# liuxinren456852/HiDeGS

Measured on AMD Instinct MI355X. Metric: binning-stage iters/sec at 2M Gaussians, 1920x1080 (scan + tile sort + ranges, the built part of the fwd+bwd iteration; the rasterizer fwd/bwd is not built: headline_metric, status), higher is better.
Workload: dtype u64/u32 (binning), f32 (distCUDA2, exchange, masked Adam)

## Files before the change

hidegs_amd/build.py:

```python
from __future__ import annotations

import concurrent.futures as cf
import glob
import hashlib
import os
import shutil
import subprocess
import sys

HERE = os.path.dirname(os.path.abspath(__file__))
CSRC = os.path.join(HERE, "csrc")
INCLUDE = os.path.join(HERE, "..", "include")
OBJDIR = os.path.join(HERE, "build")
LIB = os.path.join(HERE, "libhidegs.so")
VARIANT_DIR = os.path.join(HERE, "variants")
SOURCES = ["abi.cpp", "timing.cpp", "primitives.hip", "knn.hip", "adam.hip", "wire.hip", "rows.hip"]
HEADERS = sorted(glob.glob(os.path.join(CSRC, "*.h"))) + [os.path.join(INCLUDE, "hidegs.h"),
                                                         os.path.join(INCLUDE, "hidegs_rows.h"),
                                                         os.path.join(INCLUDE, "hidegs_resize.h"),
                                                         os.path.join(INCLUDE, "hidegs_clone.h")]

FLAGS = ["--offload-arch=gfx950", "-O3", "-std=c++17", "-fPIC", "-ffp-contract=off", "-Wall",
         "-Wno-unused-function", "-I", INCLUDE]

VARIANTS = {
    "qcap": (["-DHIDEGS_JOB_CAP=64", "-DHIDEGS_MAX_POLLS=65536u"], ["primitives.hip"]),
    "gform": (["-DHIDEGS_QUEUE_MIN=8192"], ["primitives.hip"]),
    "wscout": (["-DHIDEGS_WIDE_SCOUTS=1"], ["primitives.hip"]),
    "pcap": (["-DHIDEGS_PIECE_CAP=16"], ["primitives.hip"]),
}


def hipcc() -> str:
    for cand in (shutil.which("hipcc"), "/opt/rocm/bin/hipcc"):
        if cand and os.path.exists(cand):
            return cand
    raise RuntimeError("hipcc not found: the HIP toolchain is required to build libhidegs.so")


def _command(src: str, obj: str, defines) -> list:
    lang = ["-x", "hip"] if src.endswith(".hip") else []
    return [hipcc(), *FLAGS, *defines, *lang, "-c", src, "-o", obj + ".tmp"]


def _stamp(cmd: list) -> str:
    return hashlib.sha256(" ".join(cmd[1:-2]).encode()).hexdigest()


def _stale(obj: str, src: str, stamp: str) -> bool:
    if not os.path.exists(obj) or not os.path.exists(obj + ".cmd"):
        return True
    with open(obj + ".cmd") as f:
        if f.read().strip() != stamp:
            return True
    t = os.path.getmtime(obj)
    return any(os.path.getmtime(p) > t for p in [src, *HEADERS])


def _compile(src: str, objdir: str, defines, verbose: bool) -> str:
    obj = os.path.join(objdir, os.path.basename(src) + ".o")
    cmd = _command(src, obj, defines)
    stamp = _stamp(cmd)
    if _stale(obj, src, stamp):
        if verbose:
            print(" ".join(cmd), flush=True)
        subprocess.run(cmd, check=True)
        os.replace(obj + ".tmp", obj)
        with open(obj + ".cmd", "w") as f:
            f.write(stamp + "\n")
    return obj


def _link(objs, lib: str, verbose: bool) -> str:
    if not os.path.exists(lib) or any(os.path.getmtime(o) > os.path.getmtime(lib) for o in objs):
        tmp = lib + ".tmp"
        cmd = [hipcc(), "--offload-arch=gfx950", "-shared", "-fPIC", *objs, "-o", tmp]
        if verbose:
            print(" ".join(cmd), flush=True)
        subprocess.run(cmd, check=True)
        os.replace(tmp, lib)
    return lib


ABI_CLIENT_SRC = os.path.join(HERE, "..", "tests", "c_abi", "abi_client.cpp")
ABI_CLIENT = os.path.join(HERE, "..", "tests", "c_abi", "abi_client")


def build_abi_client(verbose: bool = False) -> str:
    deps = [ABI_CLIENT_SRC, LIB, os.path.join(INCLUDE, "hidegs.h")]
    if not os.path.exists(ABI_CLIENT) or any(os.path.getmtime(d) > os.path.getmtime(ABI_CLIENT) for d in deps):
        tmp = ABI_CLIENT + ".tmp"
        cmd = [hipcc(), "--offload-arch=gfx950", "-O2", "-std=c++17", "-ffp-contract=off", "-Wall", ABI_CLIENT_SRC,
               "-L" + HERE, "-lhidegs", "-Wl,-rpath,$ORIGIN/../../hidegs_amd", "-o", tmp]
        if verbose:
            print(" ".join(cmd), flush=True)
        subprocess.run(cmd, check=True)
        os.replace(tmp, ABI_CLIENT)
    return ABI_CLIENT


def variant_path(tag: str) -> str:
    return os.path.join(VARIANT_DIR, f"libhidegs_{tag}.so")


def _compile_all(sources, objdir: str, defines, verbose: bool) -> list:
    os.makedirs(objdir, exist_ok=True)
    with cf.ThreadPoolExecutor(max_workers=8) as ex:
        return list(ex.map(lambda s: _compile(os.path.join(CSRC, s), objdir, defines, verbose), sources))


def build_variant(tag: str, defines, changed=SOURCES, verbose: bool = False) -> str:
    objs = dict(zip(changed, _compile_all(changed, os.path.join(VARIANT_DIR, "obj_" + tag), defines, verbose)))
    rest = [s for s in SOURCES if s not in objs]
    objs.update(zip(rest, _compile_all(rest, OBJDIR, [], verbose)))
    return _link([objs[s] for s in SOURCES], variant_path(tag), verbose)


def build(verbose: bool = False, variants: bool = True) -> str:
    _link(_compile_all(SOURCES, OBJDIR, [], verbose), LIB, verbose)
    if variants:
        with cf.ThreadPoolExecutor(max_workers=len(VARIANTS)) as ex:
            list(ex.map(lambda tv: build_variant(tv[0], *tv[1], verbose=verbose), VARIANTS.items()))
        build_abi_client(verbose)
    return LIB


if __name__ == "__main__":
    print(build(verbose="-v" in sys.argv))
```

hidegs_amd/csrc/primitives.hip:

```cpp
#include "block_scan.h"
#include "common.h"

#include <mutex>

namespace hidegs {
int identify_tile_ranges(const uint64_t* keys, long long n, uint32_t* ranges, int num_tiles, hipStream_t stream);

namespace {

constexpr int kBlock = 256;
constexpr int kItems = 16;
constexpr int kTile = kBlock * kItems;
constexpr int kWavesPerBlock = kBlock / kWave;
constexpr int kRadixBits = 8;
constexpr int kRadix = 1 << kRadixBits;

#ifndef HIDEGS_SCOUTS
#define HIDEGS_SCOUTS 128
#endif

inline int ceil_div(long long a, long long b) { return (int)((a + b - 1) / b); }

#include "scan.h"
#include "radix.h"
#include "segment_forms.h"
#include "queue_trace.h"
#include "hot_queue.h"
#include "segment_sort.h"


constexpr int kRangeKeys = 4;
__global__ __launch_bounds__(kBlock) void identify_ranges_kernel(const uint64_t* __restrict__ keys, long long n,
                                                                 uint2* __restrict__ ranges, uint32_t num_tiles,
                                                                 uint32_t tile_mask)
{
    const long long i0 = ((long long)blockIdx.x * kBlock + threadIdx.x) * kRangeKeys;
    if (i0 >= n) return;
    uint32_t tile[kRangeKeys];
    if (i0 + kRangeKeys <= n && (reinterpret_cast<uintptr_t>(keys) & 15) == 0) {
        const ulonglong2* k2 = reinterpret_cast<const ulonglong2*>(keys + i0);
        const ulonglong2 a = k2[0], b = k2[1];
        tile[0] = (uint32_t)(a.x >> 32) & tile_mask;
        tile[1] = (uint32_t)(a.y >> 32) & tile_mask;
        tile[2] = (uint32_t)(b.x >> 32) & tile_mask;
        tile[3] = (uint32_t)(b.y >> 32) & tile_mask;
    } else {
#pragma unroll
        for (int j = 0; j < kRangeKeys; j++) tile[j] = i0 + j < n ? (uint32_t)(keys[i0 + j] >> 32) & tile_mask : 0u;
    }
    uint32_t prev = i0 == 0 ? 0u : (uint32_t)(keys[i0 - 1] >> 32) & tile_mask;
#pragma unroll
    for (int j = 0; j < kRangeKeys; j++) {
        const long long i = i0 + j;
        if (i >= n) break;
        const uint32_t cur = tile[j];
        if (i == 0) {
            if (cur < num_tiles) ranges[cur].x = 0;
        } else {
            if (cur != prev) {
                if (prev < num_tiles) ranges[prev].y = (uint32_t)i;
                if (cur < num_tiles) ranges[cur].x = (uint32_t)i;
            }
            if (i == n - 1 && cur < num_tiles) ranges[cur].y = (uint32_t)n;
        }
        prev = cur;
    }
}



size_t scan_scratch(long long n)
{
    const int nt = ceil_div(n, kDevScanTile);
    return align_up((size_t)nt * sizeof(uint32_t)) + align_up(sizeof(uint32_t));
}

constexpr int kMaxSegmentBits = 16;
constexpr long long kSegmentedMinN = 65536;
constexpr long long kSegmentedMinAvg = 64;
constexpr long long kTileSegmentedMinAvg = 8;

BigQueue queue_caps(long long n)
{
    BigQueue q{};
    q.rec_cap = (uint32_t)(5 * (n / (kSegCap + 1)) + 8);
#ifdef HIDEGS_JOB_CAP
    q.job_cap = (uint32_t)HIDEGS_JOB_CAP;
#else
    q.job_cap = (uint32_t)(n / 24 + 1024);
#endif
    q.pool_cap = (uint32_t)(n / 2 + 16 * kRadix);
#ifdef HIDEGS_PIECE_CAP
    q.piece_cap = (uint32_t)HIDEGS_PIECE_CAP;
#else
    q.piece_cap = (uint32_t)(n / 512 + 1024);
#endif
    return q;
}

template <typename K>
size_t sort_scratch(long long n)
{
    const int nt = ceil_div(n, kTile);
    size_t b = align_up((size_t)n * sizeof(K)) + align_up((size_t)n * sizeof(uint32_t)) +
               align_up((size_t)kRadix * nt * sizeof(uint32_t)) + 2 * align_up(kRadix * sizeof(uint32_t));
    if (sizeof(K) == 8) {
        const BigQueue q = queue_caps(n);
        b += align_up(sizeof(uint32_t) * (((size_t)1 << kMaxSegmentBits) + 1)) + align_up(kRadix * sizeof(uint32_t)) +
             align_up(Q_WORDS * sizeof(uint32_t)) +
             align_up((size_t)q.rec_cap * sizeof(BigSeg)) + align_up((size_t)q.job_cap * sizeof(uint4)) +
             align_up((size_t)q.pool_cap * sizeof(uint32_t)) + align_up((size_t)q.piece_cap * sizeof(uint2));
    }
    return b;
}

__global__ void identify_ranges_kernel(const uint64_t* __restrict__ keys, long long n, uint2* __restrict__ ranges,
                                       uint32_t num_tiles, uint32_t tile_mask);

template <typename K>
int sort_pairs(void* scratch, size_t scratch_bytes, const K* keys_in, K* keys_out, const uint32_t* vals_in,
               uint32_t* vals_out, long long n, int begin_bit, int end_bit, hipStream_t stream, const char* what,
               uint2* ranges_out = nullptr, int num_tiles = 0)
{
    const int kbits = (int)(8 * sizeof(K));
    if (n < 0 || begin_bit < 0 || end_bit > kbits || begin_bit > end_bit)
        return fail(HIDEGS_E_ARG, std::string(what) + ": bad size or bit range");
    if (n > 0x7fffffffLL) return fail(HIDEGS_E_ARG, std::string(what) + ": more than 2^31-1 items");
    if (n == 0)
        return ranges_out ? identify_tile_ranges(nullptr, 0, reinterpret_cast<uint32_t*>(ranges_out), num_tiles, stream)
                          : 0;
    if (!keys_in || !keys_out || !vals_in || !vals_out)
        return fail(HIDEGS_E_ARG, std::string(what) + ": NULL key/value pointer");
    if (keys_out == keys_in || vals_out == vals_in)
        return fail(HIDEGS_E_ARG, std::string(what) + ": in-place sorting is not supported");
    if (!scratch || scratch_bytes < sort_scratch<K>(n))
        return fail(HIDEGS_E_ARG, std::string(what) + ": scratch buffer too small");

    const int passes = (end_bit - begin_bit + kRadixBits - 1) / kRadixBits;
    if (passes == 0) {
        if (hipMemcpyAsync(keys_out, keys_in, n * sizeof(K), hipMemcpyDeviceToDevice, stream) != hipSuccess ||
            hipMemcpyAsync(vals_out, vals_in, n * sizeof(uint32_t), hipMemcpyDeviceToDevice, stream) != hipSuccess)
            return fail(HIDEGS_E_HIP, std::string(what) + ": copy failed");
        return ranges_out ? identify_tile_ranges(reinterpret_cast<const uint64_t*>(keys_out), n,
                                                 reinterpret_cast<uint32_t*>(ranges_out), num_tiles, stream)
                          : 0;
    }
    const int nt = ceil_div(n, kTile);
    Carver c(scratch);
    K* alt_k = c.take<K>(n);
    uint32_t* alt_v = c.take<uint32_t>(n);
    uint32_t* counts = c.take<uint32_t>((size_t)kRadix * nt);
    uint32_t* totals_pass[2] = {c.take<uint32_t>(kRadix), c.take<uint32_t>(kRadix)};

    const bool avg_ok = ranges_out ? n >= kTileSegmentedMinAvg * (long long)num_tiles
                                   : n >= (kSegmentedMinAvg << (end_bit - 32));
    const bool segmented = sizeof(K) == 8 && begin_bit == 0 && end_bit > 32 && end_bit - 32 <= kMaxSegmentBits &&
                           n >= kSegmentedMinN && avg_ok;
    const int lo_bit = segmented ? 32 : begin_bit;
    const int lsd_passes = segmented ? (end_bit - 32 + kRadixBits - 1) / kRadixBits : passes;

    const bool packed = segmented && ranges_out != nullptr;
    int nseg = 0;
    uint32_t* seg_starts = nullptr;
    uint32_t* low_base = nullptr;
    BigQueue q{};
    if (segmented) {
        nseg = ranges_out ? num_tiles : 1 << (end_bit - 32);
        seg_starts = c.take<uint32_t>(((size_t)1 << kMaxSegmentBits) + 1);
        low_base = c.take<uint32_t>(kRadix);
        q = queue_caps(n);
        q.ctl = c.take<uint32_t>(Q_WORDS);
        q.job = c.take<uint4>(q.job_cap);
        q.rec = c.take<BigSeg>(q.rec_cap);
        q.pool = c.take<uint32_t>(q.pool_cap);
        q.alt_k = reinterpret_cast<uint64_t*>(alt_k);
        q.alt_v = alt_v;
        q.piece = c.take<uint2>(q.piece_cap);
    }

    const K* src_k = keys_in;
    const uint32_t* src_v = vals_in;
    const int span = end_bit - lo_bit;
    int shift = lo_bit;
    int pass_bits[2] = {0, 0};
    for (int p = 0; p < lsd_passes; p++) {
        const int bits = (span * (p + 1)) / lsd_passes - (span * p) / lsd_passes;
        const uint32_t mask = (1u << bits) - 1u;
        const bool to_out = ((lsd_passes - 1 - p) % 2) == 0;
        K* dk = to_out ? keys_out : alt_k;
        uint32_t* dv = to_out ? vals_out : alt_v;
        uint32_t* totals = totals_pass[p & 1];
        const bool last = p == lsd_passes - 1;
        uint4* zero_jobs = segmented && last ? reinterpret_cast<uint4*>(q.ctl) : nullptr;
        static_assert(Q_WORDS * sizeof(uint32_t) % kAlign == 0, "ctl and job slots contiguous");
        const bool rec_in = packed && lsd_passes == 2 && last, rec_digit_out = packed && lsd_passes == 2 && !last;
        const int next_shift = shift + bits;
        const uint32_t next_mask = rec_digit_out ? (1u << (span - bits)) - 1u : 0u;
        const char* hist_name = sizeof(K) == 8 ? "radix_hist_u64" : "radix_hist_u32";
        if (rec_in)
            HIDEGS_LAUNCH(hist_name, (radix_hist_kernel<K, true>), dim3(nt), dim3(kBlock), 0, stream,
                          reinterpret_cast<const K*>(src_v), n, shift, mask, nt, counts, zero_jobs,
                          zero_jobs ? q.job_cap + Q_WORDS / 4 : 0u);
        else
            HIDEGS_LAUNCH(hist_name, radix_hist_kernel<K>, dim3(nt), dim3(kBlock), 0, stream, src_k, n, shift, mask, nt,
                          counts, zero_jobs, zero_jobs ? q.job_cap + Q_WORDS / 4 : 0u);
        const bool low = segmented && last && lsd_passes == 2;
        HIDEGS_LAUNCH("radix_digit_scan", radix_digit_scan_kernel, dim3(mask + 1), dim3(kBlock), 0, stream, counts,
                      nt, totals, low ? totals_pass[0] : nullptr, low ? 1 << pass_bits[0] : 0, low_base);
        if (p < 2) pass_bits[p] = bits;
        const bool with_starts = segmented && last;
        const int b0 = with_starts && lsd_passes == 2 ? pass_bits[0] : 0;
        const bool narrow = (int)mask < kNarrowRadix && n <= kNarrowMaxN && (1 << b0) <= kNarrowRadix;
        const char* scatter_name = sizeof(K) == 8 ? "radix_scatter_u64" : "radix_scatter_u32";
#define HIDEGS_SCATTER(...)                                                                                            \
    HIDEGS_LAUNCH(scatter_name, (radix_scatter_kernel<K, __VA_ARGS__>), dim3(nt), dim3(kSBlock), 0, stream, src_k, src_v, \
                  dk, dv, n, shift, mask, nt, counts, totals, with_starts ? low_base : nullptr, b0,                       \
                  with_starts ? seg_starts : nullptr, next_shift, next_mask)
        if (rec_in) {
            if (narrow) HIDEGS_SCATTER(true, kNarrowRadix, kOutRecords, true);
            else HIDEGS_SCATTER(true, kRadix, kOutRecords, true);
        } else if (rec_digit_out) {
            if (narrow) HIDEGS_SCATTER(false, kNarrowRadix, kOutRecordsDigit);
            else HIDEGS_SCATTER(false, kRadix, kOutRecordsDigit);
        } else if (with_starts && packed) {
            if (narrow) HIDEGS_SCATTER(true, kNarrowRadix, kOutRecords);
            else HIDEGS_SCATTER(true, kRadix, kOutRecords);
        } else if (with_starts) {
            if (narrow) HIDEGS_SCATTER(true, kNarrowRadix);
            else HIDEGS_SCATTER(true, kRadix);
        } else {
            if (narrow) HIDEGS_SCATTER(false, kNarrowRadix);
            else HIDEGS_SCATTER(false, kRadix);
        }
#undef HIDEGS_SCATTER
        src_k = dk;
        src_v = dv;
        shift += bits;
    }
    if (segmented) {
        uint64_t* ko = reinterpret_cast<uint64_t*>(keys_out);
        if (packed)
            HIDEGS_LAUNCH("segment_sort", segment_sort_kernel<true>, dim3(nseg + kScouts), dim3(kBlock), 0, stream, ko,
                          vals_out, seg_starts, ranges_out, nseg, q);
        else
            HIDEGS_LAUNCH("segment_sort", segment_sort_kernel<false>, dim3(nseg + kScouts), dim3(kBlock), 0, stream, ko,
                          vals_out, seg_starts, ranges_out, nseg, q);
        HIDEGS_LAUNCH("big_segments", big_segment_kernel, dim3(kQueueBlocks), dim3(kBlock), 0, stream, ko, vals_out,
                      reinterpret_cast<uint64_t*>(alt_k), alt_v, q);
        const bool debug = debug_enabled();
        uint32_t* async_err = debug ? nullptr : async_error_slot(stream);
        HIDEGS_LAUNCH("piece_sort", piece_sort_kernel, dim3(kPieceBlocks), dim3(kBlock), 0, stream, ko, vals_out,
                      reinterpret_cast<const uint64_t*>(alt_k), alt_v, q, async_err);
        if (debug) {
            if (int rc = check_launch(what, stream, 1)) return rc;
            uint32_t err = 0;
            if (hipMemcpyAsync(&err, q.ctl + kCtlStride * Q_ERROR, sizeof(err), hipMemcpyDeviceToHost, stream) !=
                    hipSuccess ||
                hipStreamSynchronize(stream) != hipSuccess)
                return fail(HIDEGS_E_HIP, std::string(what) + ": queue error readback failed");
            if (err)
                return fail(HIDEGS_E_HIP, std::string(what) + ": hot-tile partition queue error " + std::to_string(err) +
                                              ((err & 1u) ? " (job slots exhausted)" : "") +
                                              ((err & 4u) ? " (a worker gave up waiting)" : "") +
                                              ": the output is not sorted");
        }
    } else if (ranges_out) {
        if (int rc = check_launch(what, stream, 0)) return rc;
        return identify_tile_ranges(reinterpret_cast<const uint64_t*>(keys_out), n,
                                    reinterpret_cast<uint32_t*>(ranges_out), num_tiles, stream);
    }
    return check_launch(what, stream, 0);
}

}

__device__ uint32_t g_queue_error_read;
__global__ void queue_error_take_kernel(int clear)
{
    g_queue_error_read = clear ? __hip_atomic_exchange(&g_queue_error, 0u, __ATOMIC_RELAXED, __HIP_MEMORY_SCOPE_AGENT)
                               : __hip_atomic_load(&g_queue_error, __ATOMIC_RELAXED, __HIP_MEMORY_SCOPE_AGENT);
}

int queue_error(hipStream_t stream, int clear, uint32_t* flags)
{
    static std::mutex m;
    std::lock_guard<std::mutex> lock(m);
    uint32_t v = 0;
    hipLaunchKernelGGL(queue_error_take_kernel, dim3(1), dim3(1), 0, stream, clear);
    if (hipGetLastError() != hipSuccess ||
        hipMemcpyFromSymbolAsync(&v, HIP_SYMBOL(g_queue_error_read), sizeof(v), 0, hipMemcpyDeviceToHost, stream) !=
            hipSuccess ||
        hipStreamSynchronize(stream) != hipSuccess)
        return fail(HIDEGS_E_HIP, "queue_error: readback failed");
    if (clear) v |= take_async_bits(stream);
    *flags = v;
    return 0;
}

int inclusive_scan_u32(void* scratch, size_t scratch_bytes, const uint32_t* in, uint32_t* out, long long n,
                       hipStream_t stream)
{
    if (n < 0) return fail(HIDEGS_E_ARG, "inclusive_scan_u32: negative size");
    if (n == 0) return 0;
    if (!in || !out) return fail(HIDEGS_E_ARG, "inclusive_scan_u32: NULL pointer");
    if (!scratch || scratch_bytes < scan_scratch(n)) return fail(HIDEGS_E_ARG, "inclusive_scan_u32: scratch too small");
    const int nt = ceil_div(n, kDevScanTile);
    Carver c(scratch);
    uint32_t* sums = c.take<uint32_t>(nt);
    HIDEGS_LAUNCH("scan_reduce", scan_reduce_kernel, dim3(nt), dim3(kBlock), 0, stream, in, n, sums);
    const int own = nt <= kOwnOffsetTiles;
    if (!own)
        HIDEGS_LAUNCH("scan_small", scan_small_kernel, dim3(1), dim3(kBlock), 0, stream, sums, nt, (uint32_t*)nullptr);
    HIDEGS_LAUNCH("scan_downsweep", scan_downsweep_kernel, dim3(nt), dim3(kBlock), 0, stream, in, n, sums, own, out);
    return check_launch("inclusive_scan_u32", stream, 0);
}

size_t inclusive_scan_scratch(long long n) { return scan_scratch(n); }
size_t sort_u64_scratch(long long n) { return sort_scratch<uint64_t>(n); }
size_t sort_u32_scratch(long long n) { return sort_scratch<uint32_t>(n); }

int sort_pairs_u64(void* scratch, size_t bytes, const uint64_t* ki, uint64_t* ko, const uint32_t* vi, uint32_t* vo,
                   long long n, int b, int e, hipStream_t s)
{
    return sort_pairs<uint64_t>(scratch, bytes, ki, ko, vi, vo, n, b, e, s, "sort_pairs_u64");
}
int sort_pairs_u32(void* scratch, size_t bytes, const uint32_t* ki, uint32_t* ko, const uint32_t* vi, uint32_t* vo,
                   long long n, int b, int e, hipStream_t s)
{
    return sort_pairs<uint32_t>(scratch, bytes, ki, ko, vi, vo, n, b, e, s, "sort_pairs_u32");
}

int sort_tile_pairs(void* scratch, size_t bytes, const uint64_t* ki, uint64_t* ko, const uint32_t* vi, uint32_t* vo,
                    long long n, int num_tiles, uint32_t* ranges, hipStream_t s)
{
    if (num_tiles < 1) return fail(HIDEGS_E_ARG, "sort_tile_pairs: num_tiles must be >= 1");
    if (!ranges) return fail(HIDEGS_E_ARG, "sort_tile_pairs: NULL ranges");
    const int end = 32 + (int)(32u - (uint32_t)__builtin_clz((uint32_t)num_tiles | 1u));
    if (end > 64) return fail(HIDEGS_E_ARG, "sort_tile_pairs: too many tiles");
    return sort_pairs<uint64_t>(scratch, bytes, ki, ko, vi, vo, n, 0, end, s, "sort_tile_pairs",
                                reinterpret_cast<uint2*>(ranges), num_tiles);
}

int identify_tile_ranges(const uint64_t* keys, long long n, uint32_t* ranges, int num_tiles, hipStream_t stream)
{
    if (n < 0 || num_tiles < 0) return fail(HIDEGS_E_ARG, "identify_tile_ranges: negative size");
    if (num_tiles > 0 && !ranges) return fail(HIDEGS_E_ARG, "identify_tile_ranges: NULL ranges");
    if (num_tiles > 0 && hipMemsetAsync(ranges, 0, (size_t)num_tiles * 2 * sizeof(uint32_t), stream) != hipSuccess)
        return fail(HIDEGS_E_HIP, "identify_tile_ranges: memset failed");
    if (n == 0) return check_launch("identify_tile_ranges", stream, 0);
    if (!keys) return fail(HIDEGS_E_ARG, "identify_tile_ranges: NULL keys");
    HIDEGS_LAUNCH("identify_ranges", identify_ranges_kernel, dim3(ceil_div(n, kBlock * kRangeKeys)), dim3(kBlock), 0, stream, keys, n,
                       reinterpret_cast<uint2*>(ranges), (uint32_t)num_tiles, 0xffffffffu);
    return check_launch("identify_tile_ranges", stream, 0);
}

}

extern "C" {

size_t hidegs_scan_scratch_bytes(long long n) { return n > 0 ? hidegs::inclusive_scan_scratch(n) : 0; }
int hidegs_inclusive_scan_u32(void* scratch, size_t scratch_bytes, const uint32_t* in, uint32_t* out, long long n,
                              void* stream)
{
    if (int rc = hidegs::take_async_error("hidegs_inclusive_scan_u32", hidegs::as_stream(stream))) return rc;
    return hidegs::inclusive_scan_u32(scratch, scratch_bytes, in, out, n, hidegs::as_stream(stream));
}

size_t hidegs_sort_pairs_u64_scratch_bytes(long long n) { return n > 0 ? hidegs::sort_u64_scratch(n) : 0; }
int hidegs_sort_pairs_u64(void* scratch, size_t scratch_bytes, const uint64_t* keys_in, uint64_t* keys_out,
                          const uint32_t* vals_in, uint32_t* vals_out, long long n, int begin_bit, int end_bit,
                          void* stream)
{
    if (int rc = hidegs::take_async_error("hidegs_sort_pairs_u64", hidegs::as_stream(stream))) return rc;
    return hidegs::sort_pairs_u64(scratch, scratch_bytes, keys_in, keys_out, vals_in, vals_out, n, begin_bit, end_bit,
                                  hidegs::as_stream(stream));
}

size_t hidegs_sort_pairs_u32_scratch_bytes(long long n) { return n > 0 ? hidegs::sort_u32_scratch(n) : 0; }
int hidegs_sort_pairs_u32(void* scratch, size_t scratch_bytes, const uint32_t* keys_in, uint32_t* keys_out,
                          const uint32_t* vals_in, uint32_t* vals_out, long long n, int begin_bit, int end_bit,
                          void* stream)
{
    if (int rc = hidegs::take_async_error("hidegs_sort_pairs_u32", hidegs::as_stream(stream))) return rc;
    return hidegs::sort_pairs_u32(scratch, scratch_bytes, keys_in, keys_out, vals_in, vals_out, n, begin_bit, end_bit,
                                  hidegs::as_stream(stream));
}

int hidegs_sort_tile_pairs(void* scratch, size_t scratch_bytes, const uint64_t* keys_in, uint64_t* keys_out,
                           const uint32_t* vals_in, uint32_t* vals_out, long long n, int num_tiles, uint32_t* ranges,
                           void* stream)
{
    if (int rc = hidegs::take_async_error("hidegs_sort_tile_pairs", hidegs::as_stream(stream))) return rc;
    return hidegs::sort_tile_pairs(scratch, scratch_bytes, keys_in, keys_out, vals_in, vals_out, n, num_tiles, ranges,
                                   hidegs::as_stream(stream));
}

int hidegs_identify_tile_ranges(const uint64_t* sorted_keys, long long n, uint32_t* ranges, int num_tiles,
                                void* stream)
{
    if (int rc = hidegs::take_async_error("hidegs_identify_tile_ranges", hidegs::as_stream(stream))) return rc;
    return hidegs::identify_tile_ranges(sorted_keys, n, ranges, num_tiles, hidegs::as_stream(stream));
}

int hidegs_queue_error(void* stream, int clear, uint32_t* flags)
{
    if (!flags) return hidegs::fail(HIDEGS_E_ARG, "hidegs_queue_error: NULL flags");
    return hidegs::queue_error(hidegs::as_stream(stream), clear, flags);
}

uint32_t hidegs_higher_msb(uint32_t n)
{
    uint32_t bits = 32u - (uint32_t)__builtin_clz(n | 1u);
    return bits;
}

#ifdef HIDEGS_QUEUE_TRACE
int hidegs_debug_wide_trace(unsigned long long* host, int max_jobs)
{
    return hidegs::trace_take(hidegs::g_wtrace, hidegs::g_wtrace_n, host, max_jobs);
}

int hidegs_debug_queue_trace(unsigned long long* host, int max_jobs)
{
    return hidegs::trace_take(hidegs::g_qtrace, hidegs::g_qtrace_n, host, max_jobs);
}
#endif
}
```

hidegs_amd/csrc/radix.h:

```cpp
#pragma once


template <typename K>
__device__ __forceinline__ uint32_t digit_of(K key, int shift, uint32_t mask)
{
    return (uint32_t)(key >> shift) & mask;
}

template <typename K, int R, bool Based = false, bool LaneMask = false>
__device__ __forceinline__ void wave_rank(const K (&k)[R], const bool (&ok)[R], int shift, uint32_t mask,
                                          uint32_t* cnt, uint32_t (&rank)[R], uint32_t vary, uint32_t dbase = 0u,
                                          uint64_t* lane_mask = nullptr)
{
    if (LaneMask) {
        const uint64_t bit = 1ull << lane_id();
#pragma unroll
        for (int r = 0; r < R; r++) {
            const uint32_t d = Based ? ((((uint32_t)k[r]) - dbase) >> shift) & mask : digit_of(k[r], shift, mask);
            if (ok[r]) __hip_atomic_fetch_or(&lane_mask[d], bit, __ATOMIC_RELAXED, __HIP_MEMORY_SCOPE_WORKGROUP);
            __builtin_amdgcn_wave_barrier();
            uint64_t same = 0ull;
            uint32_t old = 0;
            if (ok[r]) {
                old = cnt[d];
                same = lane_mask[d];
            }
            __builtin_amdgcn_wave_barrier();
            const uint32_t below =
                __builtin_amdgcn_mbcnt_hi((uint32_t)(same >> 32), __builtin_amdgcn_mbcnt_lo((uint32_t)same, 0u));
            if (ok[r] && below == 0) {
                cnt[d] = old + (uint32_t)__popcll(same);
                lane_mask[d] = 0ull;
            }
            __builtin_amdgcn_wave_barrier();
            rank[r] = old + below;
        }
        return;
    }
#pragma unroll
    for (int r = 0; r < R; r++) {
        const uint32_t d = Based ? ((((uint32_t)k[r]) - dbase) >> shift) & mask : digit_of(k[r], shift, mask);
        const uint64_t okb = __ballot(ok[r]);
        uint32_t mlo = (uint32_t)okb, mhi = (uint32_t)(okb >> 32);
#pragma unroll
        for (int b = 0; b < kRadixBits; b++) {
            if (!((vary >> b) & 1u)) continue;
            const uint32_t nb = ((d >> b) & 1u) - 1u;
            const uint64_t bb = __ballot(nb == 0u);
            mlo &= nb ^ (uint32_t)bb;
            mhi &= nb ^ (uint32_t)(bb >> 32);
        }
        const uint32_t below = __builtin_amdgcn_mbcnt_hi(mhi, __builtin_amdgcn_mbcnt_lo(mlo, 0u));
        uint32_t old = 0;
        if (ok[r]) old = cnt[d];
        __builtin_amdgcn_wave_barrier();
        if (ok[r] && below == 0) cnt[d] = old + (uint32_t)(__popc(mlo) + __popc(mhi));
        __builtin_amdgcn_wave_barrier();
        rank[r] = old + below;
    }
}

__device__ __forceinline__ uint32_t digit_wave_prefix(uint32_t (*s_cnt)[kRadix])
{
    const int d = threadIdx.x;
    uint32_t run = 0;
#pragma unroll
    for (int w = 0; w < kWavesPerBlock; w++) {
        const uint32_t c = s_cnt[w][d];
        s_cnt[w][d] = run;
        run += c;
    }
    return run;
}

template <typename K, bool Bytes = false>
__global__ __launch_bounds__(kBlock) void radix_hist_kernel(const K* __restrict__ keys, long long n, int shift,
                                                            uint32_t mask, int ntiles, uint32_t* __restrict__ counts,
                                                            uint4* __restrict__ zero_jobs, uint32_t zero_count)
{
    for (uint32_t j = blockIdx.x * kBlock + threadIdx.x; j < zero_count; j += gridDim.x * kBlock)
        zero_jobs[j] = make_uint4(0u, 0u, 0u, 0u);
    __shared__ uint32_t s_hist[kWavesPerBlock][kRadix];
    const int t = threadIdx.x;
    const int wave = t / kWave;
    for (int i = t; i < kWavesPerBlock * kRadix; i += kBlock) (&s_hist[0][0])[i] = 0;
    __syncthreads();
    const int tile = xcd_swizzle(blockIdx.x, gridDim.x);
    const long long base = (long long)tile * kTile;
    K k[kItems];
    if (Bytes) {
        const uint8_t* dg = reinterpret_cast<const uint8_t*>(keys);
        static_assert(kItems == 16, "a thread's 16 digit bytes are one uint4");
        if (base + kTile <= n && (reinterpret_cast<uintptr_t>(dg) & 15) == 0) {
            const uint4 p = reinterpret_cast<const uint4*>(dg + base)[t];
            const uint32_t w[4] = {p.x, p.y, p.z, p.w};
#pragma unroll
            for (int j = 0; j < kItems; j++) atomicAdd(&s_hist[wave][(w[j / 4] >> (8 * (j % 4))) & mask], 1u);
        } else {
#pragma unroll
            for (int j = 0; j < kItems; j++) {
                const long long i = base + j * kBlock + t;
                if (i < n) atomicAdd(&s_hist[wave][dg[i] & mask], 1u);
            }
        }
    } else if (sizeof(K) == 8 && base + kTile <= n && (reinterpret_cast<uintptr_t>(keys) & 15) == 0) {
        const ulonglong2* k2 = reinterpret_cast<const ulonglong2*>(keys + base);
#pragma unroll
        for (int j = 0; j < kItems / 2; j++) {
            const ulonglong2 p = k2[j * kBlock + t];
            k[2 * j] = (K)p.x;
            k[2 * j + 1] = (K)p.y;
        }
#pragma unroll
        for (int j = 0; j < kItems; j++) atomicAdd(&s_hist[wave][digit_of(k[j], shift, mask)], 1u);
    } else {
#pragma unroll
        for (int j = 0; j < kItems; j++) {
            long long i = base + j * kBlock + t;
            k[j] = (i < n) ? keys[i] : K(0);
        }
#pragma unroll
        for (int j = 0; j < kItems; j++) {
            long long i = base + j * kBlock + t;
            if (i < n) atomicAdd(&s_hist[wave][digit_of(k[j], shift, mask)], 1u);
        }
    }
    __syncthreads();
    for (int d = t; d < kRadix; d += kBlock) {
        uint32_t c = 0;
#pragma unroll
        for (int w = 0; w < kWavesPerBlock; w++) c += s_hist[w][d];
        counts[(long long)d * ntiles + tile] = c;
    }
}

constexpr int kDigitItems = 8;
__global__ __launch_bounds__(kBlock) void radix_digit_scan_kernel(uint32_t* __restrict__ counts, int ntiles,
                                                                  uint32_t* __restrict__ totals,
                                                                  const uint32_t* __restrict__ low_totals, int nlow,
                                                                  uint32_t* __restrict__ low_base)
{
    if (low_totals && blockIdx.x == 0) {
        __shared__ uint32_t s_low[kWavesPerBlock];
        uint32_t dummy;
        const uint32_t b = block_exclusive_scan((int)threadIdx.x < nlow ? low_totals[threadIdx.x] : 0u, s_low, &dummy);
        if ((int)threadIdx.x < nlow) low_base[threadIdx.x] = b;
    }
    __shared__ uint32_t s_wave[kWavesPerBlock];
    uint32_t* row = counts + (long long)blockIdx.x * ntiles;
    uint32_t carry = 0;
    for (int base = 0; base < ntiles; base += kBlock * kDigitItems) {
        uint32_t v[kDigitItems];
        uint32_t sum = 0;
#pragma unroll
        for (int j = 0; j < kDigitItems; j++) {
            int i = base + threadIdx.x * kDigitItems + j;
            v[j] = (i < ntiles) ? row[i] : 0u;
            sum += v[j];
        }
        uint32_t total;
        uint32_t pre = block_exclusive_scan(sum, s_wave, &total) + carry;
#pragma unroll
        for (int j = 0; j < kDigitItems; j++) {
            int i = base + threadIdx.x * kDigitItems + j;
            if (i < ntiles) row[i] = pre;
            pre += v[j];
        }
        carry += total;
    }
    if (threadIdx.x == 0) totals[blockIdx.x] = carry;
}

constexpr int kSWaves = 8;
constexpr int kSBlock = kSWaves * kWave;
constexpr int kSItems = kTile / kSBlock;
static_assert(kSBlock >= kRadix, "one thread per digit in the digit scans");

template <typename K, int R, int D = kRadix>
__device__ __forceinline__ void segment_starts(const K (&k)[R], const bool (&ok)[R], const int shift, const uint32_t mask,
                                            const long long n, const int tile, const int ntiles,
                                            const long long base, const uint32_t digit_base,
                                            const uint32_t p0, const int b0, uint32_t* starts)
{
    __shared__ uint32_t s_bhist[D];
    __shared__ uint32_t s_blist[D];
    __shared__ uint32_t s_nb;
    const int t = threadIdx.x, lane = lane_id(), wave = t / kWave;
    if (t == 0) {
        s_nb = 0u;
        if (tile == 0) starts[(mask + 1u) << b0] = (uint32_t)n;
    }
    if (b0 == 0) {
        if (tile == 0 && t <= (int)mask) starts[t] = digit_base;
        return;
    }
    __syncthreads();
    if (t < (1 << b0) && (((long long)p0 >= base && (long long)p0 < base + kTile) ||
                          ((long long)p0 >= n && tile == ntiles - 1)))
        s_blist[atomicAdd(&s_nb, 1u)] = (uint32_t)t | (((uint32_t)((long long)p0 - base)) << 8);
    __syncthreads();
    const uint32_t nb = s_nb;
    for (uint32_t b = 0; b < nb; b++) {
        const uint32_t e = s_blist[b], L = e & 0xffu, r = e >> 8;
        if (t < D) s_bhist[t] = 0u;
        __syncthreads();
#pragma unroll
        for (int q = 0; q < R; q++) {
            const uint32_t li = (uint32_t)(wave * (R * kWave) + q * kWave + lane);
            if (ok[q] && li < r) atomicAdd(&s_bhist[digit_of(k[q], shift, mask)], 1u);
        }
        __syncthreads();
        if (t <= (int)mask) starts[((uint32_t)t << b0) | L] = digit_base + s_bhist[t];
        __syncthreads();
    }
}

constexpr int kNarrowRadix = 128;
constexpr long long kNarrowMaxN = 12ll << 20;
constexpr int kOutPairs = 0, kOutRecords = 1, kOutRecordsDigit = 2;
template <typename K, bool Starts = false, int D = kRadix, int Out = kOutPairs, bool RecIn = false>
__global__ __launch_bounds__(kSBlock) __attribute__((amdgpu_waves_per_eu(D == kRadix ? 1 : 8))) void radix_scatter_kernel(const K* __restrict__ keys_in,
                                                                const uint32_t* __restrict__ vals_in,
                                                                K* __restrict__ keys_out, uint32_t* __restrict__ vals_out,
                                                                long long n, int shift, uint32_t mask, int ntiles,
                                                                const uint32_t* __restrict__ tile_prefix,
                                                                const uint32_t* __restrict__ totals,
                                                                const uint32_t* __restrict__ totals0, int b0,
                                                                uint32_t* __restrict__ starts, int next_shift,
                                                                uint32_t next_mask)
{
    __shared__ __attribute__((aligned(16))) K s_stage[kTile];
    __shared__ uint32_t s_cnt[kSWaves][D];
    __shared__ uint32_t s_start[D];
    __shared__ uint32_t s_off[D];
    __shared__ uint32_t s_wave[kSWaves];
    uint32_t* s_vals = reinterpret_cast<uint32_t*>(s_stage);

    const int t = threadIdx.x;
    const int lane = lane_id();
    const int wave = __builtin_amdgcn_readfirstlane(t / kWave);
    const bool digit_thread = t < D;
    for (int i = t; i < kSWaves * D; i += kSBlock) (&s_cnt[0][0])[i] = 0;
    const int tile = xcd_swizzle(blockIdx.x, gridDim.x);
    const long long base = (long long)tile * kTile;
    const long long seg = base + (long long)wave * (kSItems * kWave);
    const uint32_t digit_total = digit_thread ? totals[t] : 0u;
    const uint32_t digit_prefix = digit_thread ? tile_prefix[(long long)t * ntiles + tile] : 0u;
    const uint32_t low_base = Starts && b0 > 0 && t < (1 << b0) ? totals0[t] : 0u;

    K k[kSItems];
    uint32_t v[kSItems];
    bool ok[kSItems];
    static_assert(!RecIn || kSItems == 8, "a lane's share of the wave's digit bytes is one 8-byte load");
    uint8_t* s_part = reinterpret_cast<uint8_t*>(s_stage) + wave * (sizeof(K) * kTile / kSWaves);
    uint8_t* s_in = s_part;
    if (RecIn) {
        const uint8_t* dg = reinterpret_cast<const uint8_t*>(vals_in);
        const long long i8 = seg + lane * 8;
        uint64_t d8 = 0ull;
        if (i8 + 8 <= n && (reinterpret_cast<uintptr_t>(dg) & 7) == 0) {
            d8 = __builtin_nontemporal_load(reinterpret_cast<const uint64_t*>(dg + i8));
        } else {
            for (int b = 0; b < 8; b++)
                if (i8 + b < n) d8 |= (uint64_t)dg[i8 + b] << (8 * b);
        }
        *reinterpret_cast<uint64_t*>(s_in + lane * 8) = d8;
        __builtin_amdgcn_wave_barrier();
    }
#pragma unroll
    for (int r = 0; r < kSItems; r++) {
        const long long i = seg + r * kWave + lane;
        ok[r] = i < n;
        if (RecIn) {
            const uint64_t rec = ok[r] ? __builtin_nontemporal_load(reinterpret_cast<const uint64_t*>(keys_in) + i) : 0ull;
            const uint32_t dg = s_in[r * kWave + lane];
            k[r] = (K)(((uint64_t)dg << shift) | (uint32_t)rec);
            v[r] = (uint32_t)(rec >> 32);
        } else {
            k[r] = ok[r] ? __builtin_nontemporal_load(keys_in + i) : K(0);
            v[r] = ok[r] ? __builtin_nontemporal_load(vals_in + i) : 0u;
        }
    }
    uint32_t dummy;
    const uint32_t digit_base = block_exclusive_scan<kSWaves>(digit_total, s_wave, &dummy) + digit_prefix;
    if (Starts) segment_starts<K, kSItems, D>(k, ok, shift, mask, n, tile, ntiles, base, digit_base, low_base, b0, starts);
    static_assert(D * sizeof(uint64_t) <= sizeof(K) * kTile / kSWaves && D % kWave == 0, "the masks fit the wave's part");
    uint64_t* s_mask = reinterpret_cast<uint64_t*>(s_part);
    __builtin_amdgcn_wave_barrier();
#pragma unroll
    for (int j = 0; j < D / kWave; j++) s_mask[j * kWave + lane] = 0ull;
    __builtin_amdgcn_wave_barrier();
    uint32_t rank[kSItems];
    wave_rank<K, kSItems, false, true>(k, ok, shift, mask, s_cnt[wave], rank, mask, 0u, s_mask);
    __syncthreads();

    uint32_t tile_count_d = 0;
    if (digit_thread) {
#pragma unroll
        for (int w = 0; w < kSWaves; w++) {
            const uint32_t c = s_cnt[w][t];
            s_cnt[w][t] = tile_count_d;
            tile_count_d += c;
        }
    }
    const uint32_t start_d = block_exclusive_scan<kSWaves>(tile_count_d, s_wave, &dummy);
    if (digit_thread) {
        s_start[t] = start_d;
        s_off[t] = digit_base - start_d;
    }
    __syncthreads();
    uint32_t pos[kSItems];
#pragma unroll
    for (int r = 0; r < kSItems; r++) {
        if (ok[r]) {
            const uint32_t dd = digit_of(k[r], shift, mask);
            pos[r] = s_start[dd] + s_cnt[wave][dd] + rank[r];
            if (Out == kOutPairs) s_stage[pos[r]] = k[r];
        }
    }
    __syncthreads();
    const int count = (int)((n - base) < kTile ? (n - base) : kTile);
    if (Out != kOutPairs) {
        static_assert(Out == kOutPairs || Starts == (Out == kOutRecords), "the last pass writes the final records");
        static_assert(sizeof(s_cnt) >= kTile && D <= 256, "a digit byte per staged position");
        uint8_t* s_digit = reinterpret_cast<uint8_t*>(&s_cnt[0][0]);
#pragma unroll
        for (int r = 0; r < kSItems; r++) {
            if (ok[r]) {
                s_stage[pos[r]] = (K)(((uint64_t)v[r] << 32) | (uint32_t)k[r]);
                s_digit[pos[r]] = (uint8_t)digit_of(k[r], shift, mask);
                if (Out == kOutRecordsDigit) pos[r] |= digit_of(k[r], next_shift, next_mask) << 16;
            }
        }
        __syncthreads();
#pragma unroll
        for (int j = 0; j < kSItems; j++) {
            const int i = t + j * kSBlock;
            if (i < count) {
                const uint32_t d = s_off[s_digit[i]] + i;
                if (d < n) keys_out[d] = s_stage[i];
            }
        }
        if (Out == kOutRecordsDigit) {
            __syncthreads();
            uint8_t* s_next = reinterpret_cast<uint8_t*>(s_stage);
            uint8_t* digits_out = reinterpret_cast<uint8_t*>(vals_out);
#pragma unroll
            for (int r = 0; r < kSItems; r++)
                if (ok[r]) s_next[pos[r] & 0xffffu] = (uint8_t)(pos[r] >> 16);
            __syncthreads();
#pragma unroll
            for (int j = 0; j < kSItems; j++) {
                const int i = t + j * kSBlock;
                if (i < count) {
                    const uint32_t d = s_off[s_digit[i]] + i;
                    if (d < n) digits_out[d] = s_next[i];
                }
            }
        }
        return;
    }
    uint32_t dst[kSItems];
#pragma unroll
    for (int j = 0; j < kSItems; j++) {
        const int i = t + j * kSBlock;
        dst[j] = 0xffffffffu;
        if (i < count) {
            const K key = s_stage[i];
            dst[j] = s_off[digit_of(key, shift, mask)] + i;
            if (dst[j] < n) keys_out[dst[j]] = key;
        }
    }
    __syncthreads();
#pragma unroll
    for (int r = 0; r < kSItems; r++)
        if (ok[r]) s_vals[pos[r]] = v[r];
    __syncthreads();
#pragma unroll
    for (int j = 0; j < kSItems; j++) {
        const int i = t + j * kSBlock;
        if (i < count && dst[j] < n) vals_out[dst[j]] = s_vals[i];
    }
}
```

Measured before the change: 6274.

## Fuse radix digit scan into span histogram and scatter via per-group total tables

```diff
diff --git a/hidegs_amd/build.py b/hidegs_amd/build.py
--- a/hidegs_amd/build.py
+++ b/hidegs_amd/build.py
@@ -28,6 +28,8 @@
     "gform": (["-DHIDEGS_QUEUE_MIN=8192"], ["primitives.hip"]),
     "wscout": (["-DHIDEGS_WIDE_SCOUTS=1"], ["primitives.hip"]),
     "pcap": (["-DHIDEGS_PIECE_CAP=16"], ["primitives.hip"]),
+    "span": (["-DHIDEGS_SPAN_TABLE_BYTES=4096", "-DHIDEGS_SPAN_MIN_GRID=1"], ["primitives.hip"]),
+    "dscan": (["-DHIDEGS_SPAN_TABLE_BYTES=0"], ["primitives.hip"]),
 }
 
 
diff --git a/hidegs_amd/csrc/primitives.hip b/hidegs_amd/csrc/primitives.hip
--- a/hidegs_amd/csrc/primitives.hip
+++ b/hidegs_amd/csrc/primitives.hip
@@ -98,12 +98,39 @@
     return q;
 }
 
+#ifndef HIDEGS_SPAN_TABLE_BYTES
+#define HIDEGS_SPAN_TABLE_BYTES 40960
+#endif
+#ifndef HIDEGS_SPAN_MIN_GRID
+#define HIDEGS_SPAN_MIN_GRID 128
+#endif
+constexpr size_t kSpanTableBytes = HIDEGS_SPAN_TABLE_BYTES;
+constexpr int kSpanMinGrid = HIDEGS_SPAN_MIN_GRID;
+constexpr int kSpanFewTiles = 4;
+constexpr size_t kSpanTrafficBytes = 8u << 20;
+
+inline SpanTable span_plan(int nt, int digits)
+{
+    SpanTable none{nullptr, 0, 0};
+    const int lanes = kSBlock / digits < kWave ? kSBlock / digits : kWave;
+    for (int S = 1; S <= kMaxSpan; S++) {
+        const int ng = ceil_div(nt, S);
+        const size_t row = (size_t)span_row_elems(ng, S) * (span_tot16(S) ? 2 : 4);
+        if (row * digits > kSpanTableBytes || ceil_div((long long)(row / 16), lanes) > kSpanLoads) continue;
+        if (row * digits * nt > kSpanTrafficBytes) continue;
+        if (S > kSpanFewTiles && ng < kSpanMinGrid) break;
+        return SpanTable{nullptr, S, ng};
+    }
+    return none;
+}
+
 template <typename K>
 size_t sort_scratch(long long n)
 {
     const int nt = ceil_div(n, kTile);
     size_t b = align_up((size_t)n * sizeof(K)) + align_up((size_t)n * sizeof(uint32_t)) +
-               align_up((size_t)kRadix * nt * sizeof(uint32_t)) + 2 * align_up(kRadix * sizeof(uint32_t));
+               align_up((size_t)kRadix * nt * sizeof(uint32_t)) + 2 * align_up(kRadix * sizeof(uint32_t)) +
+               2 * align_up(kSpanTableBytes);
     if (sizeof(K) == 8) {
         const BigQueue q = queue_caps(n);
         b += align_up(sizeof(uint32_t) * (((size_t)1 << kMaxSegmentBits) + 1)) + align_up(kRadix * sizeof(uint32_t)) +
@@ -151,6 +178,7 @@
     uint32_t* alt_v = c.take<uint32_t>(n);
     uint32_t* counts = c.take<uint32_t>((size_t)kRadix * nt);
     uint32_t* totals_pass[2] = {c.take<uint32_t>(kRadix), c.take<uint32_t>(kRadix)};
+    void* span_tot[2] = {c.take<char>(kSpanTableBytes), c.take<char>(kSpanTableBytes)};
 
     const bool avg_ok = ranges_out ? n >= kTileSegmentedMinAvg * (long long)num_tiles
                                    : n >= (kSegmentedMinAvg << (end_bit - 32));
@@ -183,6 +211,14 @@
     const int span = end_bit - lo_bit;
     int shift = lo_bit;
     int pass_bits[2] = {0, 0};
+    constexpr int kMaxPasses = (int)(8 * sizeof(K)) / kRadixBits;
+    SpanTable plan[kMaxPasses];
+    for (int p = 0; p < lsd_passes; p++) {
+        const int bits = (span * (p + 1)) / lsd_passes - (span * p) / lsd_passes;
+        plan[p] = span_plan(nt, 1 << bits);
+        plan[p].tot = span_tot[p & 1];
+    }
+    if (segmented && lsd_passes == 2 && plan[1].S == 0) plan[0].S = 0;
     for (int p = 0; p < lsd_passes; p++) {
         const int bits = (span * (p + 1)) / lsd_passes - (span * p) / lsd_passes;
         const uint32_t mask = (1u << bits) - 1u;
@@ -197,16 +233,35 @@
         const int next_shift = shift + bits;
         const uint32_t next_mask = rec_digit_out ? (1u << (span - bits)) - 1u : 0u;
         const char* hist_name = sizeof(K) == 8 ? "radix_hist_u64" : "radix_hist_u32";
-        if (rec_in)
+        const bool low = segmented && last && lsd_passes == 2;
+        const SpanTable tab = plan[p];
+        if (tab.S > 0) {
+            const SpanTable prev = low ? (plan[0].S > 0 ? plan[0] : SpanTable{totals_pass[0], 0, 0}) : SpanTable{nullptr, 0, 0};
+            const uint32_t zero_count = zero_jobs ? q.job_cap + Q_WORDS / 4 : 0u;
+#define HIDEGS_SPAN_HIST(KEYS, BYTES)                                                                                  \
+    do {                                                                                                               \
+        if (tab.S == 1)                                                                                                \
+            HIDEGS_LAUNCH(hist_name, (radix_span_hist_kernel<K, BYTES, 1, kBlock>), dim3(tab.ng), dim3(kBlock), 0, stream, \
+                          KEYS, n, shift, mask, nt, counts, tab, prev, low ? 1 << pass_bits[0] : 0,                    \
+                          low ? low_base : nullptr, zero_jobs, zero_count);                                            \
+        else                                                                                                           \
+            HIDEGS_LAUNCH(hist_name, (radix_span_hist_kernel<K, BYTES, kMaxSpan, kSpanBlock>), dim3(tab.ng),           \
+                          dim3(kSpanBlock), 0, stream, KEYS, n, shift, mask, nt, counts, tab, prev,                    \
+                          low ? 1 << pass_bits[0] : 0, low ? low_base : nullptr, zero_jobs, zero_count);               \
+    } while (0)
+            if (rec_in) HIDEGS_SPAN_HIST(reinterpret_cast<const K*>(src_v), true);
+            else HIDEGS_SPAN_HIST(src_k, false);
+#undef HIDEGS_SPAN_HIST
+        } else if (rec_in)
             HIDEGS_LAUNCH(hist_name, (radix_hist_kernel<K, true>), dim3(nt), dim3(kBlock), 0, stream,
                           reinterpret_cast<const K*>(src_v), n, shift, mask, nt, counts, zero_jobs,
                           zero_jobs ? q.job_cap + Q_WORDS / 4 : 0u);
         else
             HIDEGS_LAUNCH(hist_name, radix_hist_kernel<K>, dim3(nt), dim3(kBlock), 0, stream, src_k, n, shift, mask, nt,
                           counts, zero_jobs, zero_jobs ? q.job_cap + Q_WORDS / 4 : 0u);
-        const bool low = segmented && last && lsd_passes == 2;
-        HIDEGS_LAUNCH("radix_digit_scan", radix_digit_scan_kernel, dim3(mask + 1), dim3(kBlock), 0, stream, counts,
-                      nt, totals, low ? totals_pass[0] : nullptr, low ? 1 << pass_bits[0] : 0, low_base);
+        if (tab.S == 0)
+            HIDEGS_LAUNCH("radix_digit_scan", radix_digit_scan_kernel, dim3(mask + 1), dim3(kBlock), 0, stream, counts,
+                          nt, totals, low ? totals_pass[0] : nullptr, low ? 1 << pass_bits[0] : 0, low_base);
         if (p < 2) pass_bits[p] = bits;
         const bool with_starts = segmented && last;
         const int b0 = with_starts && lsd_passes == 2 ? pass_bits[0] : 0;
@@ -215,7 +270,7 @@
 #define HIDEGS_SCATTER(...)                                                                                            \
     HIDEGS_LAUNCH(scatter_name, (radix_scatter_kernel<K, __VA_ARGS__>), dim3(nt), dim3(kSBlock), 0, stream, src_k, src_v, \
                   dk, dv, n, shift, mask, nt, counts, totals, with_starts ? low_base : nullptr, b0,                       \
-                  with_starts ? seg_starts : nullptr, next_shift, next_mask)
+                  with_starts ? seg_starts : nullptr, next_shift, next_mask, tab)
         if (rec_in) {
             if (narrow) HIDEGS_SCATTER(true, kNarrowRadix, kOutRecords, true);
             else HIDEGS_SCATTER(true, kRadix, kOutRecords, true);
diff --git a/hidegs_amd/csrc/radix.h b/hidegs_amd/csrc/radix.h
--- a/hidegs_amd/csrc/radix.h
+++ b/hidegs_amd/csrc/radix.h
@@ -169,6 +169,159 @@
         carry += total;
     }
     if (threadIdx.x == 0) totals[blockIdx.x] = carry;
+}
+
+constexpr int kMaxSpan = 32;
+constexpr int kSpanBlock = 1024;
+constexpr int kSpanLoads = 5;
+struct SpanTable {
+    void* tot;
+    int S;
+    int ng;
+};
+__host__ __device__ inline bool span_tot16(int S) { return S * 4096 <= 65535; }
+__host__ __device__ inline int span_row_elems(int ng, int S) { return span_tot16(S) ? (ng + 7) & ~7 : (ng + 3) & ~3; }
+
+template <int L>
+__device__ __forceinline__ void span_row_sums(const SpanTable tab, int d, bool active, int sub, int G, int g,
+                                              uint32_t& total, uint32_t& part)
+{
+    const bool t16 = span_tot16(tab.S);
+    const int epc = t16 ? 8 : 4;
+    const int nchunk = span_row_elems(tab.ng, tab.S) / epc;
+    const uint4* row = reinterpret_cast<const uint4*>(tab.tot) + (long long)d * nchunk;
+    total = part = 0u;
+    for (int c0 = 0; c0 < nchunk; c0 += G * L) {
+        uint4 q[L];
+#pragma unroll
+        for (int j = 0; j < L; j++) {
+            const int c = c0 + j * G + sub;
+            q[j] = active && c < nchunk ? row[c] : make_uint4(0u, 0u, 0u, 0u);
+        }
+#pragma unroll
+        for (int j = 0; j < L; j++) {
+            const int keep = g - (c0 + j * G + sub) * epc;
+            const uint32_t w[4] = {q[j].x, q[j].y, q[j].z, q[j].w};
+#pragma unroll
+            for (int i = 0; i < 4; i++) {
+                if (t16) {
+                    const int kw = keep - 2 * i;
+                    const uint32_t m = kw >= 2 ? 0xffffffffu : kw == 1 ? 0xffffu : 0u, x = w[i] & m;
+                    total += (w[i] & 0xffffu) + (w[i] >> 16);
+                    part += (x & 0xffffu) + (x >> 16);
+                } else {
+                    total += w[i];
+                    part += keep > i ? w[i] : 0u;
+                }
+            }
+        }
+    }
+}
+
+template <int U, int BT, typename V, typename LoadF, typename UseF>
+__device__ __forceinline__ void span_stream(int count, int t, LoadF load, UseF use)
+{
+    for (int b = 0; b < count; b += U * BT) {
+        V p[U];
+#pragma unroll
+        for (int j = 0; j < U; j++) {
+            const int i = b + j * BT + t;
+            p[j] = V{};
+            if (i < count) p[j] = load(i);
+        }
+#pragma unroll
+        for (int j = 0; j < U; j++) {
+            const int i = b + j * BT + t;
+            if (i < count) use(i, p[j]);
+        }
+    }
+}
+
+template <typename K, bool Bytes, int MaxS, int BT>
+__global__ __launch_bounds__(BT) void radix_span_hist_kernel(const K* __restrict__ keys, long long n, int shift,
+                                                             uint32_t mask, int ntiles, uint32_t* __restrict__ counts,
+                                                             SpanTable tab, SpanTable low, int nlow,
+                                                             uint32_t* __restrict__ low_base,
+                                                             uint4* __restrict__ zero_jobs, uint32_t zero_count)
+{
+    static_assert(BT % kRadix == 0 && MaxS <= kMaxSpan, "thread d owns digit d; whole lane groups per digit");
+    for (uint32_t j = blockIdx.x * BT + threadIdx.x; j < zero_count; j += gridDim.x * BT)
+        zero_jobs[j] = make_uint4(0u, 0u, 0u, 0u);
+    __shared__ uint32_t s_hist[MaxS][kRadix];
+    __shared__ uint32_t s_low[kRadix];
+    __shared__ uint32_t s_wave[BT / kWave];
+    const int t = threadIdx.x;
+    const int S = tab.S;
+    for (int i = t; i < S * kRadix; i += BT) (&s_hist[0][0])[i] = 0;
+    if (low_base && blockIdx.x == 0) {
+        int G = BT / nlow;
+        G = G > kWave ? kWave : G;
+        const int d = t / G, sub = t % G;
+        uint32_t sum = 0, dummy;
+        if (low.S == 0) {
+            sum = sub == 0 && d < nlow ? reinterpret_cast<const uint32_t*>(low.tot)[d] : 0u;
+        } else {
+            span_row_sums<2>(low, d, d < nlow, sub, G, 0, sum, dummy);
+            for (int o = 1; o < G; o <<= 1) sum += wave_shfl_xor(sum, o);
+        }
+        if (sub == 0 && d < nlow) s_low[d] = sum;
+        __syncthreads();
+        const uint32_t b = block_exclusive_scan<BT / kWave>(t < nlow ? s_low[t] : 0u, s_wave, &dummy);
+        if (t < nlow) low_base[t] = b;
+    }
+    __syncthreads();
+    const int g = xcd_swizzle(blockIdx.x, gridDim.x);
+    const long long lo = (long long)g * S * kTile;
+    const int count = (int)((n - lo) < (long long)S * kTile ? (n - lo) : (long long)S * kTile);
+    int done = 0;
+    if (Bytes) {
+        const uint8_t* dg = reinterpret_cast<const uint8_t*>(keys) + lo;
+        if ((reinterpret_cast<uintptr_t>(dg) & 15) == 0) {
+            const uint4* p4 = reinterpret_cast<const uint4*>(dg);
+            span_stream<4, BT, uint4>(
+                count >> 4, t, [&](int i) { return p4[i]; },
+                [&](int i, const uint4& p) {
+                    uint32_t* h = s_hist[i >> 8];
+                    const uint32_t w[4] = {p.x, p.y, p.z, p.w};
+#pragma unroll
+                    for (int j = 0; j < 16; j++) atomicAdd(&h[(w[j / 4] >> (8 * (j % 4))) & mask], 1u);
+                });
+            done = (count >> 4) << 4;
+        }
+        for (int i = done + t; i < count; i += BT) atomicAdd(&s_hist[i >> 12][dg[i] & mask], 1u);
+    } else {
+        const K* kp = keys + lo;
+        if (sizeof(K) == 8 && (reinterpret_cast<uintptr_t>(kp) & 15) == 0) {
+            const ulonglong2* k2 = reinterpret_cast<const ulonglong2*>(kp);
+            span_stream<8, BT, ulonglong2>(
+                count >> 1, t, [&](int i) { return k2[i]; },
+                [&](int i, const ulonglong2& p) {
+                    uint32_t* h = s_hist[i >> 11];
+                    atomicAdd(&h[digit_of((K)p.x, shift, mask)], 1u);
+                    atomicAdd(&h[digit_of((K)p.y, shift, mask)], 1u);
+                });
+            done = (count >> 1) << 1;
+        }
+        span_stream<8, BT, K>(
+            count - done, t, [&](int i) { return kp[done + i]; },
+            [&](int i, const K& key) { atomicAdd(&s_hist[(done + i) >> 12][digit_of(key, shift, mask)], 1u); });
+    }
+    __syncthreads();
+    if (t < kRadix && t <= (int)mask) {
+        uint32_t run = 0;
+        const int tile0 = g * S;
+        for (int s = 0; s < S && tile0 + s < ntiles; s++) {
+            counts[(long long)t * ntiles + tile0 + s] = run;
+            run += s_hist[s][t];
+        }
+        const int stride = span_row_elems(tab.ng, S);
+        const int end = g == tab.ng - 1 ? stride : g + 1;
+        for (int i = g; i < end; i++) {
+            const uint32_t v = i == g ? run : 0u;
+            if (span_tot16(S)) reinterpret_cast<uint16_t*>(tab.tot)[(long long)t * stride + i] = (uint16_t)v;
+            else reinterpret_cast<uint32_t*>(tab.tot)[(long long)t * stride + i] = v;
+        }
+    }
 }
 
 constexpr int kSWaves = 8;
@@ -227,7 +380,7 @@
                                                                 const uint32_t* __restrict__ totals,
                                                                 const uint32_t* __restrict__ totals0, int b0,
                                                                 uint32_t* __restrict__ starts, int next_shift,
-                                                                uint32_t next_mask)
+                                                                uint32_t next_mask, SpanTable span)
 {
     __shared__ __attribute__((aligned(16))) K s_stage[kTile];
     __shared__ uint32_t s_cnt[kSWaves][D];
@@ -244,8 +397,17 @@
     const int tile = xcd_swizzle(blockIdx.x, gridDim.x);
     const long long base = (long long)tile * kTile;
     const long long seg = base + (long long)wave * (kSItems * kWave);
-    const uint32_t digit_total = digit_thread ? totals[t] : 0u;
-    const uint32_t digit_prefix = digit_thread ? tile_prefix[(long long)t * ntiles + tile] : 0u;
+    uint32_t digit_total = 0u, row_total = 0u, row_part = 0u;
+    const int gbits = 9 - __popc(mask) < 6 ? 9 - __popc(mask) : 6;
+    static_assert(kSBlock == 1 << 9 && kSBlock / kWave <= kNarrowRadix, "the lane groups' digits fit every instance");
+    if (span.S > 0) {
+        const int d = t >> gbits;
+        span_row_sums<kSpanLoads>(span, d, d <= (int)mask, t & ((1 << gbits) - 1), 1 << gbits, tile / span.S, row_total,
+                                  row_part);
+    } else {
+        digit_total = digit_thread ? totals[t] : 0u;
+    }
+    uint32_t digit_prefix = digit_thread ? tile_prefix[(long long)t * ntiles + tile] : 0u;
     const uint32_t low_base = Starts && b0 > 0 && t < (1 << b0) ? totals0[t] : 0u;
 
     K k[kSItems];
@@ -282,6 +444,21 @@
         }
     }
     uint32_t dummy;
+    if (span.S > 0) {
+        for (int o = 1; o < (1 << gbits); o <<= 1) {
+            row_total += wave_shfl_xor(row_total, o);
+            row_part += wave_shfl_xor(row_part, o);
+        }
+        if ((t & ((1 << gbits) - 1)) == 0) {
+            s_start[t >> gbits] = row_total;
+            s_off[t >> gbits] = row_part;
+        }
+        __syncthreads();
+        if (digit_thread && t <= (int)mask) {
+            digit_total = s_start[t];
+            digit_prefix += s_off[t];
+        }
+    }
     const uint32_t digit_base = block_exclusive_scan<kSWaves>(digit_total, s_wave, &dummy) + digit_prefix;
     if (Starts) segment_starts<K, kSItems, D>(k, ok, shift, mask, n, tile, ntiles, base, digit_base, low_base, b0, starts);
     static_assert(D * sizeof(uint64_t) <= sizeof(K) * kTile / kSWaves && D % kWave == 0, "the masks fit the wave's part");
```

Result: no change. 6313 (median of 6 runs) (+0.6%).
